# robbert-vdh/haskell-path-tracer

Measured on AMD Instinct MI355X. Metric: Msamples/sec (paths×bounces) at 1080p/64spp; achieved HBM GB/s vs peak, higher is better.
Workload: dtype f32

## Files before the change

### haskell-path-tracer_amd/_build.py

```python
import hashlib
import mmap
import os
import shutil
import subprocess
from concurrent.futures import ThreadPoolExecutor

HERE = os.path.dirname(os.path.abspath(__file__))
ROOT = os.path.dirname(HERE)
CSRC = os.path.join(HERE, "csrc")
LIB = os.path.join(HERE, "libptmi.so")
ABLATIONS_LIB = os.path.join(HERE, "libptmi_ablations.so")
OBJ_ROOT = os.path.join(ROOT, "build", "obj")
HOST_SOURCES = ["ptmi_api.cpp", "ptmi_stage.cpp", "ptmi_group.cpp", "ptmi_bvh.cpp", "ptmi_mesh.cpp"]
BUILD_ID_UNIT = "ptmi_build_id.cpp"
BUILD_ID_MARKER = b"PTMI_BUILD_ID="
SOURCE_HASH_MARKER = b"PTMI_SOURCE_HASH="
INLINE_UNIT = "ptmi_inline.hip"
KERNEL_UNITS = [INLINE_UNIT, "ptmi_streams_chain.hip", "ptmi_streams_tree.hip", "ptmi_stream_primary.hip", "ptmi_stream_pixels.hip",
                "ptmi_stream_split.hip", "ptmi_small.hip", "ptmi_mesh_refit.hip", "ptmi_mesh_build.hip", "ptmi_bvh_refit.hip", "ptmi_bvh_build.hip", "ptmi_bvh_lbvh.hip"]
ABLATION_UNITS = ["ptmi_inline_ablations.hip"]
SOURCES = HOST_SOURCES + [BUILD_ID_UNIT] + KERNEL_UNITS + ABLATION_UNITS
HEADERS = ["ptmi_core.h", "ptmi_kernels.h", "ptmi_device.h", "ptmi_bvh_device.h", "ptmi_bvh.h", "ptmi_bvh_box.h", "ptmi_bvh_spatial.h", "ptmi_mesh_device.h", "ptmi_mesh.h", "ptmi_mesh_box.h", "ptmi_mesh_morton.h", "ptmi_inline_body.inc", "ptmi_streams_chain_body.inc", "ptmi_streams_tree_body.inc", "ptmi_diag.h", "ptmi_stream_form.h", "ptmi_stage.h",
           os.path.join("..", "..", "include", "ptmi.h")]
COMPILE_FLAGS = ["--offload-arch=gfx950", "-O3", "-std=c++17", "-ffp-contract=off", "-fPIC",
                 "-fno-fast-math", "-fno-slp-vectorize", "-DPTMI_SINCOS_FUSED=1", "-Wall", "-pthread"]
LINK_FLAGS = ["--offload-arch=gfx950", "-shared", "-fPIC", "-pthread", "-ldl"]
FLAGS = COMPILE_FLAGS + ["-shared", "-ldl"]
RECIPE = "cwd=csrc,cuid=unit+flags"
JOBS = max(1, min(8, os.cpu_count() or 1))


def hipcc_path():
    for cand in (os.environ.get("HIPCC"), shutil.which("hipcc"), "/opt/rocm/bin/hipcc"):
        if cand and os.path.exists(cand):
            return cand
    raise RuntimeError("hipcc not found; libptmi.so cannot be built")


def source_hash():
    h = hashlib.sha256(" ".join(COMPILE_FLAGS + LINK_FLAGS + [RECIPE]).encode())
    for f in sorted(SOURCES + HEADERS):
        with open(os.path.join(CSRC, f), "rb") as fh:
            h.update(f.encode() + b"\0" + fh.read())
    return h.hexdigest()[:16]


def object_code_hash(obj):
    with open(obj, "rb") as fh:
        data = fh.read()
    if data[:4] != b"\x7fELF" or data[4] != 2 or data[5] != 1:
        raise RuntimeError("%s is not a little-endian ELF64 object" % obj)
    shoff = int.from_bytes(data[0x28:0x30], "little")
    shentsize, shnum, shstrndx = (int.from_bytes(data[o:o + 2], "little") for o in (0x3A, 0x3C, 0x3E))

    def header(i):
        b = data[shoff + i * shentsize: shoff + (i + 1) * shentsize]
        return (int.from_bytes(b[0:4], "little"), int.from_bytes(b[4:8], "little"), int.from_bytes(b[8:16], "little"),
                int.from_bytes(b[24:32], "little"), int.from_bytes(b[32:40], "little"))
    _, _, _, str_off, str_size = header(shstrndx)
    names = data[str_off:str_off + str_size]
    h = hashlib.sha256()
    for i in range(shnum):
        name, typ, flags, off, size = header(i)
        if not flags & 2 or typ == 8:
            continue
        h.update(names[name:names.index(b"\0", name)] + b"\0" + size.to_bytes(8, "little") + data[off:off + size])
    return h.hexdigest()


def code_id_of(objs):
    h = hashlib.sha256()
    for obj in sorted(objs, key=os.path.basename):
        h.update(os.path.basename(obj).encode() + b"\0" + object_code_hash(obj).encode() + b"\0")
    return h.hexdigest()[:16]

# ... 184 lines not shown
```

### haskell-path-tracer_amd/csrc/ptmi_core.h

```cpp
#pragma once

#include <hip/hip_runtime.h>
#include <stdint.h>

#define PTMI_HD __host__ __device__ __forceinline__

namespace ptmi {

struct V3 { float x, y, z; };
struct Quat { float w; V3 v; };
struct Sfc32 { uint32_t a, b, c, counter; };

constexpr float kPi       = 3.14159274101257324219f;
constexpr float kInfinite = 3.40282346638528859812e+38f;
constexpr float kEpsilon  = 0.002f;

PTMI_HD uint32_t f2u(float f) { return __builtin_bit_cast(uint32_t, f); }
PTMI_HD float u2f(uint32_t u) { return __builtin_bit_cast(float, u); }

PTMI_HD V3 mk(float x, float y, float z) { V3 r; r.x = x; r.y = y; r.z = z; return r; }
PTMI_HD V3 operator+(V3 a, V3 b) { return mk(a.x + b.x, a.y + b.y, a.z + b.z); }
PTMI_HD V3 operator-(V3 a, V3 b) { return mk(a.x - b.x, a.y - b.y, a.z - b.z); }
PTMI_HD V3 operator*(V3 a, V3 b) { return mk(a.x * b.x, a.y * b.y, a.z * b.z); }
PTMI_HD V3 neg(V3 a) { return mk(-a.x, -a.y, -a.z); }
PTMI_HD V3 scale_r(V3 v, float a) { return mk(v.x * a, v.y * a, v.z * a); }
PTMI_HD V3 scale_l(float a, V3 v) { return mk(a * v.x, a * v.y, a * v.z); }
PTMI_HD V3 div_r(V3 v, float a) { return mk(v.x / a, v.y / a, v.z / a); }
PTMI_HD float dot(V3 a, V3 b) { return (a.x * b.x + a.y * b.y) + a.z * b.z; }
PTMI_HD V3 cross(V3 a, V3 b)
{
    return mk(a.y * b.z - a.z * b.y, a.z * b.x - a.x * b.z, a.x * b.y - a.y * b.x);
}
PTMI_HD bool near_zero(float a) { return __builtin_fabsf(a) <= 1e-6f; }
PTMI_HD bool near_zero(V3 v) { return near_zero(dot(v, v)); }
PTMI_HD V3 normalize(V3 v)
{
    float l = dot(v, v);
    if (near_zero(l) || near_zero(1.0f - l)) return v;
    return div_r(v, __builtin_sqrtf(l));
}
PTMI_HD Quat qmul(Quat a, Quat b)
{
    Quat r;
    r.w = a.w * b.w - dot(a.v, b.v);
    r.v = (cross(a.v, b.v) + scale_l(a.w, b.v)) + scale_l(b.w, a.v);
    return r;
}
PTMI_HD V3 rotate(Quat q, V3 v)
{
    Quat qv; qv.w = 0.0f; qv.v = v;
    Quat qc; qc.w = q.w; qc.v = neg(q.v);
    return qmul(qmul(q, qv), qc).v;
}

struct Reduced { double x; int n; };
__host__ __device__ __noinline__ inline Reduced sincos_reduce_large(uint32_t xi)
{
    constexpr uint32_t inv_pio4[24] = {
        0xa2,       0xa2f9,     0xa2f983,   0xa2f9836e, 0xf9836e4e, 0x836e4e44,
        0x6e4e4415, 0x4e441529, 0x441529fc, 0x1529fc27, 0x29fc2757, 0xfc2757d1,
        0x2757d1f5, 0x57d1f534, 0xd1f534dd, 0xf534ddc0, 0x34ddc0db, 0xddc0db62,
        0xc0db6295, 0xdb629599, 0x6295993c, 0x95993c43, 0x993c4390, 0x3c439041 };
    const int base = (xi >> 26) & 15;
    const int shift = (xi >> 23) & 7;
    xi = (xi & 0xffffff) | 0x800000;
    xi <<= shift;
    uint64_t res0 = (uint32_t)(xi * inv_pio4[base]);
    uint64_t res1 = (uint64_t)xi * inv_pio4[base + 4];
    uint64_t res2 = (uint64_t)xi * inv_pio4[base + 8];
    res0 = (res2 >> 32) | (res0 << 32);
    res0 += res1;
    uint64_t n = (res0 + (1ULL << 61)) >> 62;
    res0 -= n << 62;
    Reduced r;
    r.x = (double)(int64_t)res0 * 0x1.921FB54442D18p-62;
    r.n = (int)n;
    return r;
}

PTMI_HD double local_constant(double k)
{
#if defined(__HIP_DEVICE_COMPILE__)
    uint32_t lo = (uint32_t)__builtin_bit_cast(uint64_t, k), hi = (uint32_t)(__builtin_bit_cast(uint64_t, k) >> 32);
    asm volatile("" : "+v"(lo), "+v"(hi));
    return __builtin_bit_cast(double, ((uint64_t)hi << 32) | lo);
// ... 210 lines not shown
```

### haskell-path-tracer_amd/csrc/ptmi_device.h

```cpp
#pragma once

#include "ptmi_kernels.h"
#include "ptmi_diag.h"

namespace ptmi {

namespace {

constexpr int kBlock = 256;
constexpr size_t kMaxSceneLds = 3 * 1024;
constexpr int kRenderBlock = 64;

struct HitSel { float t; int idx; bool just; };
#ifdef PTMI_NO_STAGED_WALK_OTHERS
constexpr bool kStagedWalk = false;
#else
constexpr bool kStagedWalk = true;
#endif

__device__ __forceinline__ float sqrt_rn(float x)
{
    const bool tiny = (f2u(x) - 1u) < (0x0f800000u - 1u);
    if (__builtin_expect(__any(tiny), 0)) return __builtin_sqrtf(x);
    const float s = __builtin_amdgcn_sqrtf(x);
    const float s_dn = u2f(f2u(s) - 1u), s_up = u2f(f2u(s) + 1u);
    const float e_dn = __builtin_fmaf(-s_dn, s, x);
    const float e_up = __builtin_fmaf(-s_up, s, x);
    float r = (e_dn <= 0.0f) ? s_dn : s;
    r = (e_up > 0.0f) ? s_up : r;
    return r;
}

__device__ __forceinline__ V3 div3_by_length(V3 v, float s)
{
#ifdef PTMI_PLAIN_DIVISION
    return div_r(v, s);
#else
    const float amin = __builtin_fminf(__builtin_fminf(__builtin_fabsf(v.x), __builtin_fabsf(v.y)), __builtin_fabsf(v.z));
    const bool plain = s >= 0x1p-20f && s <= 0x1p20f && amin >= 0x1p-100f;
    if (__builtin_expect(!__all(plain), 0)) return div_r(v, s);
    const float r0 = __builtin_amdgcn_rcpf(s);
    const float r = __builtin_fmaf(__builtin_fmaf(-s, r0, 1.0f), r0, r0);
    auto quotient = [&](float a) {
        float q = a * r;
        q = __builtin_fmaf(__builtin_fmaf(-s, q, a), r, q);
        return __builtin_fmaf(__builtin_fmaf(-s, q, a), r, q);
    };
    return mk(quotient(v.x), quotient(v.y), quotient(v.z));
#endif
}

template <typename ScenePtr>
__device__ __noinline__ HitSel check_hit_exact(ScenePtr S, int ns, int np, V3 o, V3 d)
{
    HitSel best; best.t = 0.0f; best.idx = 0; best.just = false;
    float best_key = 0.0f;
    for (int i = 0; i < ns + np; ++i) {
        bool just; float t;
        if (i < ns) {
            const float4 g = S[i];
            const V3 l = mk(g.x, g.y, g.z) - o;
            const float tca = dot(l, d);
            const float d2 = dot(l, l) - (tca * tca);
            const float thc = __builtin_sqrtf(g.w - d2);
            t = tca - thc;
            just = !(tca < 0.0f || d2 > g.w || t < 0.0f);
        } else {
            const float4 gp = S[ns + 2 * (i - ns)], gn = S[ns + 2 * (i - ns) + 1];
            const V3 nor = mk(gn.x, gn.y, gn.z);
            const float denom = dot(d, nor);
            t = dot(mk(gp.x, gp.y, gp.z) - o, nor) / denom;
            just = !(denom > 1e-6f || t < 0.0f);
        }
        const float key = just ? t : kInfinite;
        if (i == 0 || !(best_key <= key)) { best_key = key; best.t = t; best.idx = i; best.just = just; }
    }
    return best;
}

#define PTMI_SPHERE_TEST(g, o, d)                                                                                                   \
    const V3 l = mk(g.x, g.y, g.z) - o;                                                                                             \
    const float tca = dot(l, d);                                                                                                    \
    const float d2 = dot(l, l) - (tca * tca);                                                                                       \
    const float x = g.w - d2;                                                       \
                             \
    const bool cand = !(tca < 0.0f) && !(x < 0.0f)

template <typename At>
__device__ __forceinline__ void fold_planes(At at, int ns, int np, V3 o, V3 d, float &best_key, int &best_idx, bool &best_just,
                                            unsigned int *diag = nullptr)
{
    int stash = 0;
    float stash_denom = 1.0f;
    unsigned long long stashed = 0ull;
    auto pass = [&]() {
        diag::plane_pass(diag);
        const float4 gp = at(2 * stash), gn = at(2 * stash + 1);
        const float t = dot(mk(gp.x, gp.y, gp.z) - o, mk(gn.x, gn.y, gn.z)) / stash_denom;
        const bool just = !(stash_denom > 1e-6f) && !(t < 0.0f);
        const float key = just ? t : kInfinite;
        if (!(best_key <= key)) { best_key = key; best_idx = ns + stash; best_just = just; }
        stash_denom = 1.0f;
        stashed = 0ull;
    };
    for (int j = 0; j < np; ++j) {
        const float4 gn = at(2 * j + 1);
        const float denom = dot(d, mk(gn.x, gn.y, gn.z));
        const bool cand = !(denom > 1e-6f);
        const unsigned long long cands = __ballot(cand);
        diag::plane_test(diag);
        if (cands & stashed) pass();
        stash = cand ? j : stash;
        stash_denom = cand ? denom : stash_denom;
        stashed |= cands;
    }
    if (stashed) pass();
}

template <bool STAGED = false, typename ScenePtr>
__device__ __forceinline__ HitSel check_hit(ScenePtr S, int ns, int np, V3 o, V3 d, unsigned int *diag = nullptr)
{
    float best_key = __builtin_nanf("");
    int best_idx = 0;
    bool best_just = false;

    auto sphere = [&](const float4 g, int i) {
        PTMI_SPHERE_TEST(g, o, d);
        diag::sphere_test(diag, cand);
        if (__any(cand)) {
            const float t = tca - sqrt_rn(x);
            const bool just = cand && !(t < 0.0f);
            const float key = just ? t : kInfinite;
            if (!(best_key <= key)) { best_key = key; best_idx = i; best_just = just; }
        }
    };

    float4 ga, gb;
    int i = 0;
#if defined(__HIP_DEVICE_COMPILE__)
    typedef __attribute__((address_space(3))) const float4 *Staged;
    Staged P = nullptr;
    if constexpr (STAGED) {
        unsigned int lds_at = (unsigned int)(uintptr_t)&S[0];
        asm volatile("" : "+v"(lds_at));
        P = (Staged)(uintptr_t)lds_at;
        ga = P[0];
        for (; i + 3 < ns; i += 4) {
            gb = P[1]; sphere(ga, i);
            ga = P[2]; sphere(gb, i + 1);
            gb = P[3]; sphere(ga, i + 2);
            ga = P[4]; sphere(gb, i + 3);
            P += 4;
        }
        for (; i + 1 < ns; i += 2) {
            gb = P[1]; sphere(ga, i);
            ga = P[2]; sphere(gb, i + 1);
            P += 2;
        }
        if (i < ns) {
            sphere(ga, i);
            P += 1;
        }
    } else
#endif
    {
        ga = S[0];
        for (; i + 1 < ns; i += 2) {
            gb = S[i + 1];
            sphere(ga, i);
            ga = S[i + 2];
            sphere(gb, i + 1);
        }
        if (i < ns) sphere(ga, i);
    }
    fold_planes([&](int k) -> float4 {
#if defined(__HIP_DEVICE_COMPILE__)
        if constexpr (STAGED) return P[k]; else
#endif
        return S[ns + k];
    }, ns, np, o, d, best_key, best_idx, best_just, diag);
    if (__builtin_expect(__any(best_just && !(best_key < kInfinite)), 0))
        return check_hit_exact(S, ns, np, o, d);
    HitSel best; best.t = best_key; best.idx = best_idx; best.just = best_just;
    return best;
}

template <typename ScenePtr>
__device__ __forceinline__ void hit_record(ScenePtr S, int ns, int idx, V3 o, V3 d, float t,
                                           V3 &hit_pos, V3 &normal)
{
    hit_pos = o + scale_r(d, t);
    if (idx < ns) {
        const float4 g = S[idx];
        const V3 v = hit_pos - mk(g.x, g.y, g.z);
        const float len2 = dot(v, v);
        normal = (near_zero(len2) || near_zero(1.0f - len2)) ? v : div3_by_length(v, sqrt_rn(len2));
    } else {
        const float4 gn = S[ns + 2 * (idx - ns) + 1];
        normal = mk(gn.x, gn.y, gn.z);
    }
}

template <typename ScenePtr>
__device__ __forceinline__ V3 normal_at(ScenePtr S, int ns, int idx, V3 hit_pos)
{
    if (idx < ns) {
        const float4 g = S[idx];
        const V3 v = hit_pos - mk(g.x, g.y, g.z);
        const float len2 = dot(v, v);
        return (near_zero(len2) || near_zero(1.0f - len2)) ? v : div3_by_length(v, sqrt_rn(len2));
    }
    const float4 gn = S[ns + 2 * (idx - ns) + 1];
    return mk(gn.x, gn.y, gn.z);
}

__device__ __forceinline__ float gen_component(Sfc32 &seed)
{
    const float i = (float)(int32_t)sfc32_next(seed);
    return ((i * 4.656612873077392578125e-10f + 1.0f) + 2.3283064365386962890625e-10f) - 1.0f;
}

__device__ __forceinline__ void bounce_axis(float4 mb, V3 normal, V3 d, V3 &axis, float &hk)
{
    const bool matte = f2u(mb.x) == 0u;
    const float ia = dot(d, normal);
    const V3 reflection = d - scale_l(2.0f * ia, normal);
    axis = matte ? normal : reflection;
    hk = matte ? 0.5f * kPi : mb.w;
}

__device__ __forceinline__ void next_about_axis(float4 mb, V3 axis, float hk, Sfc32 &seed, V3 &next, float &brdf)
{
    const bool matte = f2u(mb.x) == 0u;
    V3 rv;
    rv.x = gen_component(seed); rv.y = gen_component(seed); rv.z = gen_component(seed);
    next = rotate(quaternion_from_half_angles(hk * rv.x, hk * rv.y, hk * rv.z), axis);
    const float nd = dot(next, axis);
    brdf = matte ? mb.z * nd : __builtin_fmaxf(0.0f, nd);
}

// ... 276 lines not shown
```

### haskell-path-tracer_amd/csrc/ptmi_inline.hip

```cpp
#include "ptmi_mesh_device.h"

namespace ptmi {

namespace {

#ifndef PTMI_INLINE_WAVES
#define PTMI_INLINE_WAVES 7
#endif
template <bool LDS_SCENE, int TILE_W = 0>
__global__ void __launch_bounds__(kRenderBlock, PTMI_INLINE_WAVES) render_inline_kernel(const RenderArgs a)
{
#define PTMI_HIT(STAGED, ...) check_hit<STAGED>(__VA_ARGS__)
#define PTMI_HIT_RECORD hit_record
#define PTMI_NORMAL_AT normal_at
#include "ptmi_inline_body.inc"
#undef PTMI_HIT_RECORD
#undef PTMI_NORMAL_AT
#undef PTMI_HIT
}

#ifndef PTMI_CONTRACTED_BUILD
template <int TILE_W>
__global__ void __launch_bounds__(kRenderBlock, PTMI_BVH_WAVES) render_inline_bvh_kernel(const RenderArgs a, const BvhView bvh)
{
    constexpr bool LDS_SCENE = false;
#define PTMI_HIT(STAGED, S, ns, np, o, d, ...) check_hit_bvh(bvh, S, ns, np, o, d)
#define PTMI_HIT_RECORD hit_record
#define PTMI_NORMAL_AT normal_at
#include "ptmi_inline_body.inc"
#undef PTMI_HIT_RECORD
#undef PTMI_NORMAL_AT
#undef PTMI_HIT
}

template <int TILE_W>
__global__ void __launch_bounds__(kRenderBlock, PTMI_BVH_WAVES) render_inline_mesh_kernel(const RenderArgs a, const MeshView mesh)
{
    constexpr bool LDS_SCENE = false;
#define PTMI_HIT(STAGED, S, ns, np, o, d, ...) check_hit_mesh(mesh, S, ns, np, o, d)
#define PTMI_HIT_RECORD(S, ns, idx, o, d, t, p, n) mesh_hit_record(mesh, S, ns, np, idx, o, d, t, p, n)
#define PTMI_NORMAL_AT(S, ns, idx, p) mesh_normal_at(mesh, S, ns, np, idx, p)
#include "ptmi_inline_body.inc"
#undef PTMI_HIT_RECORD
#undef PTMI_NORMAL_AT
#undef PTMI_HIT
}
#endif

hipError_t launch_linear(const RenderArgs &a, Mapping mapping, bool lds_scene, hipStream_t stream)
{
    if (lds_scene) return launch_per_pixel(a, mapping, render_inline_kernel<true, 8>, render_inline_kernel<true>, true, PTMI_INLINE_WAVES, 16, stream);
    return launch_per_pixel(a, mapping, render_inline_kernel<false, 8>, render_inline_kernel<false>, false, PTMI_INLINE_WAVES, 16, stream);
}

}

hipError_t launch_render_inline(const RenderArgs &a, const BvhView *bvh, int variant, hipStream_t stream)
{
    if (renders_nothing(a)) return hipSuccess;
#ifndef PTMI_CONTRACTED_BUILD
    if (bvh) return launch_per_pixel(a, Mapping::kAuto, render_inline_bvh_kernel<8>, render_inline_bvh_kernel<0>, false, PTMI_BVH_WAVES, 16, stream, *bvh);
#endif
    const bool lds_scene = scene_fits_lds(a);
    if (variant == kVariantAuto || a.bounce_limit <= 0 || a.n_spp <= 0) return launch_linear(a, Mapping::kAuto, lds_scene, stream);
    if (!lds_scene) {
        if (variant == kVariantPersistent) variant = kVariantPersistentScalar;
        else if (variant == kVariantRows || variant == kVariantCapped4 || variant == kVariantCapped3) variant = kVariantRowsScalar;
        else if (variant >= kVariantTiles && variant <= kVariantTiles32x2) variant = kVariantTilesScalar;
// ... 55 lines not shown
```

### haskell-path-tracer_amd/csrc/ptmi_inline_body.inc

```
    __shared__ float pixel_const[10][kRenderBlock];
    extern __shared__ float4 lds_scene[];
    const int ns = a.scene.n_spheres, np = a.scene.n_planes;
    if (LDS_SCENE) {
        const int total = a.scene.total_f4();
        for (int i = threadIdx.x; i < total; i += kRenderBlock) lds_scene[i] = a.scene.packed[i];
        __syncthreads();
    }
    const float4 *S = LDS_SCENE ? lds_scene : a.scene.packed;
    const float4 *M = S + a.scene.geom_f4();

    unsigned int wg; int chunk, n_spp_chunk;
    enter_sample_chunk<TILE_W>(a, wg, chunk, n_spp_chunk);
    long long pixel;
    unsigned int quad, trips = 0;
    const bool valid = lane_pixel<TILE_W>(a, pixel, quad, wg);
    unsigned int live = 0;
    if (valid) {
        const int local_row = (int)(pixel / a.width);
        const int col = (int)(pixel - (long long)local_row * a.width);
        int64_t px = col, py = global_row(local_row, a.stripe_rows, a.n_parts, a.part);
        if (a.screen_x) { px = a.screen_x[pixel]; py = a.screen_y[pixel]; }

        const V3 origin = a.cam.pos;
        const V3 primary = primary_direction(a.cam, px, py);

        V3 acc = mk(a.planes.r[pixel], a.planes.g[pixel], a.planes.b[pixel]);
        Sfc32 seed;
        seed.a = a.planes.sa[pixel]; seed.b = a.planes.sb[pixel];
        seed.c = a.planes.sc[pixel]; seed.counter = a.planes.sctr[pixel];

        const int limit = a.bounce_limit, n_spp = n_spp_chunk;

        if (limit <= 0) {
            if (n_spp > 0) acc = mk(0.0f, 0.0f, 0.0f) + acc;
        } else {
            const HitSel h0 = PTMI_HIT(LDS_SCENE, S, ns, np, origin, primary);
            if (!h0.just) {
                if (n_spp > 0) acc = mk(0.0f, 0.0f, 0.0f) + acc;
            } else {
                float *mine = &pixel_const[0][threadIdx.x];
                auto put = [&](int k, float v) { mine[k * kRenderBlock] = v; };
                auto get = [&](int k) { return mine[k * kRenderBlock]; };
                V3 pos, normal;
                PTMI_HIT_RECORD(S, ns, h0.idx, origin, primary, h0.t, pos, normal);
                const int idx0 = h0.idx;
                {
                    const float4 mb0 = M[2 * idx0 + 1];
                    V3 axis0; float hk0;
                    bounce_axis(mb0, normal, primary, axis0, hk0);
                    put(0, pos.x); put(1, pos.y); put(2, pos.z);
                    put(3, axis0.x); put(4, axis0.y); put(5, axis0.z); put(6, hk0);
                    put(7, acc.x); put(8, acc.y); put(9, acc.z);
                }
                int s = -1, it = 0, idx = idx0;
                V3 d = primary;
                V3 throughput = mk(1.0f, 1.0f, 1.0f), result = mk(0.0f, 0.0f, 0.0f);
                bool pending = false, has_ray = false, over = n_spp > 0;
                diag::PhaseProbe phase;
                while (pending || over) {
                    ++trips;
                    phase.trip(); phase.round_a(pending || over);
                    float4 mb = M[2 * idx + 1];
                    V3 axis = mk(0.0f, 0.0f, 0.0f); float hk = 0.0f;
                    phase.check(pending);
                    if (pending) {
                        bounce_axis(mb, normal, d, axis, hk);
                        const float4 ma = M[2 * idx];
                        if (it + 1 >= limit || surely_frozen_after(ma, mb, axis, throughput)) {
                            finish_frozen(ma, throughput, result, seed);
                            ++live;
                            phase.frozen();
                            pending = false; over = true;
                        }
                    }
                    phase.restart(over);
                    if (over) {
                        if (s >= 0) { put(7, result.x + get(7)); put(8, result.y + get(8)); put(9, result.z + get(9)); }
                        ++s; it = 0;
                        throughput = mk(1.0f, 1.0f, 1.0f); result = mk(0.0f, 0.0f, 0.0f);
                        pos = mk(get(0), get(1), get(2)); idx = idx0;
                        mb = M[2 * idx0 + 1];
                        axis = mk(get(3), get(4), get(5)); hk = get(6);
                        over = false; pending = s < n_spp;
                    }
                    phase.shade(pending);
                    if (pending) {
                        V3 next; float brdf;
                        sincos3_probe(a.work_counter, hk, seed);
                        next_about_axis(mb, axis, hk, seed, next, brdf);
                        apply_bounce(M, idx, pos, next, brdf, pos, d, throughput, result);
                        ++it; ++live;
                        pending = false;
                        if (it >= limit || near_zero(throughput)) over = true;
                        else has_ray = true;
                    }
                    phase.end_a(); phase.round_c(has_ray);
                    if (has_ray) {
                        const HitSel h = PTMI_HIT(LDS_SCENE, S, ns, np, pos, d, diag::sphere_counters(a.work_counter));
                        has_ray = false;
                        if (h.just) {
                            PTMI_HIT_RECORD(S, ns, h.idx, pos, d, h.t, pos, normal);
                            idx = h.idx;
                            pending = true;
                        } else {
                            over = true;
                        }
                    }
                    phase.end_c();
                }
                acc = mk(get(7), get(8), get(9));
                phase.flush(a.work_counter);
            }
        }

        a.planes.r[pixel] = acc.x; a.planes.g[pixel] = acc.y; a.planes.b[pixel] = acc.z;
        a.planes.sa[pixel] = seed.a; a.planes.sb[pixel] = seed.b;
        a.planes.sc[pixel] = seed.c; a.planes.sctr[pixel] = seed.counter;
    }
    leave_sample_chunk<TILE_W>(a, wg, chunk);

    if (TILE_W > 0) record_cost(a, quad, trips);
    if (a.live_counter) {
        const unsigned long long total = wave_sum(live);
        if ((threadIdx.x & 63) == 0 && total) atomicAdd(a.live_counter + (size_t)(blockIdx.x & (kStatShards - 1)) * kStatStride, total);
    }
```

### haskell-path-tracer_amd/csrc/ptmi_small.hip

```cpp
#include "ptmi_mesh_device.h"

namespace ptmi {

namespace {

__global__ void __launch_bounds__(kBlock) seed_kernel(Planes p, int width, int rows_local, int stripe_rows,
                                                      int n_parts, int part, uint64_t seed0, int clear_color)
{
    const long long n_local = (long long)rows_local * width;
    const long long pixel = (long long)blockIdx.x * kBlock + threadIdx.x;
    if (pixel >= n_local) return;
    const int local_row = (int)(pixel / width);
    const int col = (int)(pixel - (long long)local_row * width);
    const uint64_t index = (uint64_t)global_row(local_row, stripe_rows, n_parts, part) * (uint64_t)width + (uint64_t)col;
    const Sfc32 s = sfc32_seed3(seed_word(seed0, index, 0), seed_word(seed0, index, 1), seed_word(seed0, index, 2));
    p.sa[pixel] = s.a; p.sb[pixel] = s.b; p.sc[pixel] = s.c; p.sctr[pixel] = s.counter;
    if (clear_color) { p.r[pixel] = 0.0f; p.g[pixel] = 0.0f; p.b[pixel] = 0.0f; }
}

__global__ void __launch_bounds__(kBlock) create_with_kernel(Planes p, const uint32_t *w0, const uint32_t *w1,
                                                             const uint32_t *w2, long long n)
{
    const long long i = (long long)blockIdx.x * kBlock + threadIdx.x;
    if (i >= n) return;
// ... 32 lines not shown
            o[2] = float4{b[2], r[3], g[3], b[3]};
        }
        if (rgba) {
            uint4 v;
            v.x = unorm8(r[0]) | unorm8(g[0]) << 8 | unorm8(b[0]) << 16 | 0xff000000u;
            v.y = unorm8(r[1]) | unorm8(g[1]) << 8 | unorm8(b[1]) << 16 | 0xff000000u;
            v.z = unorm8(r[2]) | unorm8(g[2]) << 8 | unorm8(b[2]) << 16 | 0xff000000u;
            v.w = unorm8(r[3]) | unorm8(g[3]) << 8 | unorm8(b[3]) << 16 | 0xff000000u;
            *reinterpret_cast<uint4 *>(rgba + q) = v;
        }
    } else {
        for (int k = 0; k < 4 && q + k < n; ++k) {
            if (rgb) { rgb[3 * (q + k)] = r[k]; rgb[3 * (q + k) + 1] = g[k]; rgb[3 * (q + k) + 2] = b[k]; }
            if (rgba) rgba[q + k] = unorm8(r[k]) | unorm8(g[k]) << 8 | unorm8(b[k]) << 16 | 0xff000000u;
        }
    }
}

__global__ void __launch_bounds__(kBlock) stitch_kernel(const float *src, int rows, int width, int stripe_rows, int n_parts, int part,
                                                        float *r, float *g, float *b)
{
    const long long n = (long long)rows * width;
    const long long i = (long long)blockIdx.x * kBlock + threadIdx.x;
    if (i >= n) return;
    const int local_row = (int)(i / width);
    const int col = (int)(i - (long long)local_row * width);
    const long long o = (long long)global_row(local_row, stripe_rows, n_parts, part) * width + col;
    r[o] = src[i]; g[o] = src[n + i]; b[o] = src[2 * n + i];
}

__global__ void __launch_bounds__(kBlock) eval_sphere_kernel(const float *sph, const float *rays, int n,
                                                             int32_t *is_just, float *t_out, float *normalp)
{
    const int i = blockIdx.x * kBlock + threadIdx.x;
    if (i >= n) return;
    const float *s = sph + 10 * (size_t)i;
    float4 g[2]; g[0].x = s[0]; g[0].y = s[1]; g[0].z = s[2]; g[0].w = s[3] * s[3];
    g[1] = g[0];
    const V3 o = mk(rays[6 * i], rays[6 * i + 1], rays[6 * i + 2]);
    const V3 d = mk(rays[6 * i + 3], rays[6 * i + 4], rays[6 * i + 5]);
    const HitSel h = check_hit(g, 1, 0, o, d);
    is_just[i] = h.just ? 1 : 0;
    t_out[i] = h.just ? h.t : 0.0f;
    if (normalp) {
        V3 hp = mk(0, 0, 0), nr = mk(0, 0, 0);
        if (h.just) hit_record(g, 1, 0, o, d, h.t, hp, nr);
        float *q = normalp + 6 * (size_t)i;
        q[0] = hp.x; q[1] = hp.y; q[2] = hp.z; q[3] = nr.x; q[4] = nr.y; q[5] = nr.z;
    }
}

template <bool BVH>
__global__ void __launch_bounds__(kRenderBlock) eval_check_hit_kernel(const SceneView scene, const BvhView bvh, const float *rays, int n,
                                                                      float *t_out, int32_t *idx_out, int32_t *just_out)
{
    const int i = blockIdx.x * kRenderBlock + threadIdx.x;
    if (i >= n) return;
    const V3 o = mk(rays[6 * (size_t)i], rays[6 * (size_t)i + 1], rays[6 * (size_t)i + 2]);
    const V3 d = mk(rays[6 * (size_t)i + 3], rays[6 * (size_t)i + 4], rays[6 * (size_t)i + 5]);
    const HitSel h = BVH ? check_hit_bvh(bvh, scene.packed, scene.n_spheres, scene.n_planes, o, d)
                         : check_hit(scene.packed, scene.n_spheres, scene.n_planes, o, d);
    just_out[i] = h.just ? 1 : 0;
    t_out[i] = h.just ? h.t : 0.0f;
    idx_out[i] = h.just ? h.idx : -1;
}

__global__ void __launch_bounds__(kRenderBlock) eval_check_hit_mesh_kernel(const SceneView scene, const MeshView mesh, const float *rays, int n,
                                                                           float *t_out, int32_t *idx_out, int32_t *just_out)
{
    const int i = blockIdx.x * kRenderBlock + threadIdx.x;
    if (i >= n) return;
    const V3 o = mk(rays[6 * (size_t)i], rays[6 * (size_t)i + 1], rays[6 * (size_t)i + 2]);
    const V3 d = mk(rays[6 * (size_t)i + 3], rays[6 * (size_t)i + 4], rays[6 * (size_t)i + 5]);
    const HitSel h = check_hit_mesh(mesh, scene.packed, scene.n_spheres, scene.n_planes, o, d);
    just_out[i] = h.just ? 1 : 0;
    t_out[i] = h.just ? h.t : 0.0f;
    idx_out[i] = h.just ? h.idx : -1;
}

__global__ void __launch_bounds__(kBlock) eval_plane_kernel(const float *pl, const float *rays, int n,
                                                            int32_t *is_just, float *t_out, float *normalp)
{
    const int i = blockIdx.x * kBlock + threadIdx.x;
    if (i >= n) return;
    const float *s = pl + 12 * (size_t)i;
    float4 g[3];
    g[0].x = s[0]; g[0].y = s[1]; g[0].z = s[2]; g[0].w = 0.0f;
    g[1].x = s[3]; g[1].y = s[4]; g[1].z = s[5]; g[1].w = 0.0f;
    g[2] = g[0];
    const V3 o = mk(rays[6 * i], rays[6 * i + 1], rays[6 * i + 2]);
    const V3 d = mk(rays[6 * i + 3], rays[6 * i + 4], rays[6 * i + 5]);
    const HitSel h = check_hit(g, 0, 1, o, d);
    is_just[i] = h.just ? 1 : 0;
    t_out[i] = h.just ? h.t : 0.0f;
    if (normalp) {
        V3 hp = mk(0, 0, 0), nr = mk(0, 0, 0);
        if (h.just) hit_record(g, 0, 0, o, d, h.t, hp, nr);
        float *q = normalp + 6 * (size_t)i;
        q[0] = hp.x; q[1] = hp.y; q[2] = hp.z; q[3] = nr.x; q[4] = nr.y; q[5] = nr.z;
    }
}

__global__ void __launch_bounds__(kBlock) eval_sincos_kernel(const float *x, int n, float *s, float *c)
{
    const int i = blockIdx.x * kBlock + threadIdx.x;
    if (i >= n) return;
    float sn, cs;
    sincos(x[i], sn, cs);
    s[i] = sn; c[i] = cs;
// ... 40 lines not shown
            unsigned int t = (cut < 256 && total) ? start[cut] : n;
            t = (t + 7u) & ~7u;
            *tail_start = t < n ? t : n;
        }
    }
    __syncthreads();
    for (unsigned int i = threadIdx.x; i < n; i += 1024) order[atomicAdd(&start[cls[i]], 1u)] = i;
}

}

bool uses_quad_order(const RenderArgs &a, int algorithm_inline, int variant)
{
    if (variant != kVariantAuto || !tiles_pay(a) || a.screen_x) return false;
    return algorithm_inline ? (a.bounce_limit > 0 && a.n_spp > 0) : true;
}


hipError_t launch_quad_order(const unsigned int *cost, unsigned int *order, unsigned int *cls, unsigned int n, unsigned int *tail_start,
                             unsigned int tail_permille, hipStream_t stream)
{
    if (n == 0) return hipSuccess;
    return launch(quad_order_kernel, dim3(1), dim3(1024), 0, stream, cost, order, cls, n, tail_start, tail_permille);
}


hipError_t launch_seed(Planes p, int width, int rows_local, int stripe_rows, int n_parts, int part,
                       uint64_t seed0, bool clear_color, hipStream_t stream)
{
    const long long n = (long long)rows_local * width;
    if (n <= 0) return hipSuccess;
    return launch(seed_kernel, dim3(blocks_for(n)), dim3(kBlock), 0, stream, p, width, rows_local,
                  stripe_rows, n_parts, part, seed0, clear_color ? 1 : 0);
}

hipError_t launch_create_with(Planes p, const uint32_t *w0, const uint32_t *w1, const uint32_t *w2,
                              int64_t n, hipStream_t stream)
{
    if (n <= 0) return hipSuccess;
    return launch(create_with_kernel, dim3(blocks_for(n)), dim3(kBlock), 0, stream, p, w0, w1, w2, (long long)n);
}

hipError_t launch_eval_sphere(const float *spheres10, const float *rays, int n,
                              int32_t *is_just, float *t, float *normalp, hipStream_t stream)
{
    if (n <= 0) return hipSuccess;
    return launch(eval_sphere_kernel, dim3(blocks_for(n)), dim3(kBlock), 0, stream, spheres10, rays, n, is_just, t, normalp);
}

hipError_t launch_eval_check_hit(SceneView scene, const BvhView *bvh, const float *rays, int n, float *t, int32_t *idx, int32_t *just, hipStream_t stream)
{
    if (n <= 0) return hipSuccess;
    const dim3 grid(blocks_for(n, kRenderBlock)), block(kRenderBlock);
    if (bvh) return launch(eval_check_hit_kernel<true>, grid, block, 0, stream, scene, *bvh, rays, n, t, idx, just);
    return launch(eval_check_hit_kernel<false>, grid, block, 0, stream, scene, BvhView{}, rays, n, t, idx, just);
}

hipError_t launch_eval_check_hit_mesh(SceneView scene, const MeshView &mesh, const float *rays, int n, float *t, int32_t *idx, int32_t *just, hipStream_t stream)
{
    if (n <= 0) return hipSuccess;
    return launch(eval_check_hit_mesh_kernel, dim3(blocks_for(n, kRenderBlock)), dim3(kRenderBlock), 0, stream, scene, mesh, rays, n, t, idx, just);
}

hipError_t launch_eval_plane(const float *planes12, const float *rays, int n,
                             int32_t *is_just, float *t, float *normalp, hipStream_t stream)
{
    if (n <= 0) return hipSuccess;
    return launch(eval_plane_kernel, dim3(blocks_for(n)), dim3(kBlock), 0, stream, planes12, rays, n, is_just, t, normalp);
}

hipError_t launch_present(Planes p, long long n, int iterations, float *rgb, uint32_t *rgba, hipStream_t stream)
{
    if (n <= 0) return hipSuccess;
    const uintptr_t bits = (uintptr_t)p.r | (uintptr_t)p.g | (uintptr_t)p.b | (uintptr_t)rgb | (uintptr_t)rgba;
    return launch(present_kernel, dim3(blocks_for((n + 3) / 4)), dim3(kBlock), 0, stream, p, n, (float)iterations, rgb, rgba,
                  (bits & 15u) == 0 ? 1 : 0);
}

hipError_t launch_stitch(const float *src, int rows, int width, int stripe_rows, int n_parts, int part,
                         float *r, float *g, float *b, hipStream_t stream)
{
    const long long n = (long long)rows * width;
    if (n <= 0) return hipSuccess;
    return launch(stitch_kernel, dim3(blocks_for(n)), dim3(kBlock), 0, stream, src, rows, width, stripe_rows, n_parts, part, r, g, b);
}

hipError_t launch_eval_sincos(const float *x, int n, float *s, float *c, hipStream_t stream)
{
    if (n <= 0) return hipSuccess;
    return launch(eval_sincos_kernel, dim3(blocks_for(n)), dim3(kBlock), 0, stream, x, n, s, c);
}

hipError_t launch_eval_quaternion(const float *half_angles, int n, float *q_out, hipStream_t stream)
{
    if (n <= 0) return hipSuccess;
    return launch(eval_quaternion_kernel, dim3(blocks_for(n)), dim3(kBlock), 0, stream, half_angles, n, q_out);
}


}
```

Measured before the change: 392,100.

## Add wave-wide MFMA sphere culling vote before per-ray sphere tests

Adds a conservative sphere culling pass that uses MFMA 16x16x4 f32 matrix ops to evaluate, for each sphere (up to 16), whether any ray in the wave could hit it. Only spheres the wave votes for are then tested per ray, with a fallback to the exact path when precision bounds are not met. The inline kernel's bounce loop is restructured into a wave-uniform loop so the wave-level vote can run each trip. The aim is to cut per-ray sphere intersection ALU work, at the cost of extra MFMA, permlane and ballot work every trip and possibly more divergence handling.

```diff
diff --git a/haskell-path-tracer_amd/_build.py b/haskell-path-tracer_amd/_build.py
--- a/haskell-path-tracer_amd/_build.py
+++ b/haskell-path-tracer_amd/_build.py
@@ -20,7 +20,7 @@
                 "ptmi_stream_split.hip", "ptmi_small.hip", "ptmi_mesh_refit.hip", "ptmi_mesh_build.hip", "ptmi_bvh_refit.hip", "ptmi_bvh_build.hip", "ptmi_bvh_lbvh.hip"]
 ABLATION_UNITS = ["ptmi_inline_ablations.hip"]
 SOURCES = HOST_SOURCES + [BUILD_ID_UNIT] + KERNEL_UNITS + ABLATION_UNITS
-HEADERS = ["ptmi_core.h", "ptmi_kernels.h", "ptmi_device.h", "ptmi_bvh_device.h", "ptmi_bvh.h", "ptmi_bvh_box.h", "ptmi_bvh_spatial.h", "ptmi_mesh_device.h", "ptmi_mesh.h", "ptmi_mesh_box.h", "ptmi_mesh_morton.h", "ptmi_inline_body.inc", "ptmi_streams_chain_body.inc", "ptmi_streams_tree_body.inc", "ptmi_diag.h", "ptmi_stream_form.h", "ptmi_stage.h",
+HEADERS = ["ptmi_core.h", "ptmi_kernels.h", "ptmi_device.h", "ptmi_bvh_device.h", "ptmi_bvh.h", "ptmi_bvh_box.h", "ptmi_bvh_spatial.h", "ptmi_mesh_device.h", "ptmi_mesh.h", "ptmi_mesh_box.h", "ptmi_mesh_morton.h", "ptmi_inline_body.inc", "ptmi_inline_trip.inc", "ptmi_sphere_cull.h", "ptmi_streams_chain_body.inc", "ptmi_streams_tree_body.inc", "ptmi_diag.h", "ptmi_stream_form.h", "ptmi_stage.h",
            os.path.join("..", "..", "include", "ptmi.h")]
 COMPILE_FLAGS = ["--offload-arch=gfx950", "-O3", "-std=c++17", "-ffp-contract=off", "-fPIC",
                  "-fno-fast-math", "-fno-slp-vectorize", "-DPTMI_SINCOS_FUSED=1", "-Wall", "-pthread"]
diff --git a/haskell-path-tracer_amd/csrc/ptmi_core.h b/haskell-path-tracer_amd/csrc/ptmi_core.h
--- a/haskell-path-tracer_amd/csrc/ptmi_core.h
+++ b/haskell-path-tracer_amd/csrc/ptmi_core.h
@@ -31,6 +31,14 @@
 {
     return mk(a.y * b.z - a.z * b.y, a.z * b.x - a.x * b.z, a.x * b.y - a.y * b.x);
 }
+#define PTMI_SPHERE_TEST(g, o, d)                                                                                                   \
+    const V3 l = mk(g.x, g.y, g.z) - o;                                                                                             \
+    const float tca = dot(l, d);                                                                                                    \
+    const float d2 = dot(l, l) - (tca * tca);                                                                                       \
+    const float x = g.w - d2;                                                       \
+                             \
+    const bool cand = !(tca < 0.0f) && !(x < 0.0f)
+
 PTMI_HD bool near_zero(float a) { return __builtin_fabsf(a) <= 1e-6f; }
 PTMI_HD bool near_zero(V3 v) { return near_zero(dot(v, v)); }
 PTMI_HD V3 normalize(V3 v)
diff --git a/haskell-path-tracer_amd/csrc/ptmi_device.h b/haskell-path-tracer_amd/csrc/ptmi_device.h
--- a/haskell-path-tracer_amd/csrc/ptmi_device.h
+++ b/haskell-path-tracer_amd/csrc/ptmi_device.h
@@ -2,6 +2,7 @@
 
 #include "ptmi_kernels.h"
 #include "ptmi_diag.h"
+#include "ptmi_sphere_cull.h"
 
 namespace ptmi {
 
@@ -78,13 +79,6 @@
     return best;
 }
 
-#define PTMI_SPHERE_TEST(g, o, d)                                                                                                   \
-    const V3 l = mk(g.x, g.y, g.z) - o;                                                                                             \
-    const float tca = dot(l, d);                                                                                                    \
-    const float d2 = dot(l, l) - (tca * tca);                                                                                       \
-    const float x = g.w - d2;                                                       \
-                             \
-    const bool cand = !(tca < 0.0f) && !(x < 0.0f)
 
 template <typename At>
 __device__ __forceinline__ void fold_planes(At at, int ns, int np, V3 o, V3 d, float &best_key, int &best_idx, bool &best_just,
@@ -186,6 +180,33 @@
 }
 
 template <typename ScenePtr>
+__device__ __forceinline__ HitSel check_hit_survivors(ScenePtr S, int ns, int np, V3 o, V3 d, unsigned int survivors, unsigned int *diag = nullptr)
+{
+    float best_key = __builtin_nanf("");
+    int best_idx = 0;
+    bool best_just = false;
+    unsigned int left = __builtin_amdgcn_readfirstlane(survivors);
+    while (left) {
+        const int i = __builtin_ctz(left);
+        left &= left - 1u;
+        const float4 g = S[i];
+        PTMI_SPHERE_TEST(g, o, d);
+        diag::sphere_test(diag, cand);
+        if (__any(cand)) {
+            const float t = tca - sqrt_rn(x);
+            const bool just = cand && !(t < 0.0f);
+            const float key = just ? t : kInfinite;
+            if (!(best_key <= key)) { best_key = key; best_idx = i; best_just = just; }
+        }
+    }
+    fold_planes([&](int k) -> float4 { return S[ns + k]; }, ns, np, o, d, best_key, best_idx, best_just, diag);
+    if (__builtin_expect(__any(best_just && !(best_key < kInfinite)), 0))
+        return check_hit_exact(S, ns, np, o, d);
+    HitSel best; best.t = best_key; best.idx = best_idx; best.just = best_just;
+    return best;
+}
+
+template <typename ScenePtr>
 __device__ __forceinline__ void hit_record(ScenePtr S, int ns, int idx, V3 o, V3 d, float t,
                                            V3 &hit_pos, V3 &normal)
 {
diff --git a/haskell-path-tracer_amd/csrc/ptmi_inline.hip b/haskell-path-tracer_amd/csrc/ptmi_inline.hip
--- a/haskell-path-tracer_amd/csrc/ptmi_inline.hip
+++ b/haskell-path-tracer_amd/csrc/ptmi_inline.hip
@@ -13,7 +13,20 @@
 #define PTMI_HIT(STAGED, ...) check_hit<STAGED>(__VA_ARGS__)
 #define PTMI_HIT_RECORD hit_record
 #define PTMI_NORMAL_AT normal_at
+#ifndef PTMI_NESTED_LOOP
+#define PTMI_UNIFORM_LOOP
+#if !defined(PTMI_CONTRACTED_BUILD) && !defined(PTMI_NO_SPHERE_CULL)
+#define PTMI_SPHERE_CULL
+#define PTMI_TRACE_VOTE(o, d, has_ray) const unsigned int cull_vote = sphere_cull_vote(S, ns, cull_scene, o, d, has_ray)
+#define PTMI_HIT_BOUNCE(STAGED, S, ns, np, o, d, dg) \
+    ((cull_vote & kCullRefused) ? check_hit<STAGED>(S, ns, np, o, d, dg) : check_hit_survivors(S, ns, np, o, d, cull_vote, dg))
+#endif
+#endif
 #include "ptmi_inline_body.inc"
+#undef PTMI_TRACE_VOTE
+#undef PTMI_HIT_BOUNCE
+#undef PTMI_SPHERE_CULL
+#undef PTMI_UNIFORM_LOOP
 #undef PTMI_HIT_RECORD
 #undef PTMI_NORMAL_AT
 #undef PTMI_HIT
diff --git a/haskell-path-tracer_amd/csrc/ptmi_inline_body.inc b/haskell-path-tracer_amd/csrc/ptmi_inline_body.inc
--- a/haskell-path-tracer_amd/csrc/ptmi_inline_body.inc
+++ b/haskell-path-tracer_amd/csrc/ptmi_inline_body.inc
@@ -1,3 +1,11 @@
+#ifndef PTMI_TRACE_VOTE
+#define PTMI_TRACE_VOTE(o, d, has_ray)
+#define PTMI_TRACE_VOTE_DEFAULTED
+#endif
+#ifndef PTMI_HIT_BOUNCE
+#define PTMI_HIT_BOUNCE PTMI_HIT
+#define PTMI_HIT_BOUNCE_DEFAULTED
+#endif
     __shared__ float pixel_const[10][kRenderBlock];
     extern __shared__ float4 lds_scene[];
     const int ns = a.scene.n_spheres, np = a.scene.n_planes;
@@ -8,12 +16,81 @@
     }
     const float4 *S = LDS_SCENE ? lds_scene : a.scene.packed;
     const float4 *M = S + a.scene.geom_f4();
+#ifdef PTMI_SPHERE_CULL
+    CullScene cull_scene = cull_scene_none();
+    if (LDS_SCENE && ns >= 1 && ns <= kCullSpheres) cull_scene = cull_stage(S, ns);
+#endif
 
     unsigned int wg; int chunk, n_spp_chunk;
     enter_sample_chunk<TILE_W>(a, wg, chunk, n_spp_chunk);
     long long pixel;
     unsigned int quad, trips = 0;
     const bool valid = lane_pixel<TILE_W>(a, pixel, quad, wg);
+#ifdef PTMI_UNIFORM_LOOP
+    unsigned int live = 0;
+    const int limit = a.bounce_limit, n_spp = n_spp_chunk;
+    V3 acc = mk(0.0f, 0.0f, 0.0f);
+    Sfc32 seed; seed.a = seed.b = seed.c = seed.counter = 0u;
+    float *mine = &pixel_const[0][threadIdx.x];
+    auto put = [&](int k, float v) { mine[k * kRenderBlock] = v; };
+    auto get = [&](int k) { return mine[k * kRenderBlock]; };
+    V3 pos = mk(0.0f, 0.0f, 0.0f), normal = mk(0.0f, 0.0f, 0.0f), d = mk(0.0f, 0.0f, 1.0f);
+    int idx0 = 0;
+    bool run = false;
+    if (valid) {
+        const int local_row = (int)(pixel / a.width);
+        const int col = (int)(pixel - (long long)local_row * a.width);
+        int64_t px = col, py = global_row(local_row, a.stripe_rows, a.n_parts, a.part);
+        if (a.screen_x) { px = a.screen_x[pixel]; py = a.screen_y[pixel]; }
+
+        const V3 origin = a.cam.pos;
+        const V3 primary = primary_direction(a.cam, px, py);
+
+        acc = mk(a.planes.r[pixel], a.planes.g[pixel], a.planes.b[pixel]);
+        seed.a = a.planes.sa[pixel]; seed.b = a.planes.sb[pixel];
+        seed.c = a.planes.sc[pixel]; seed.counter = a.planes.sctr[pixel];
+
+        if (limit <= 0) {
+            if (n_spp > 0) acc = mk(0.0f, 0.0f, 0.0f) + acc;
+        } else {
+            const HitSel h0 = PTMI_HIT(LDS_SCENE, S, ns, np, origin, primary);
+            if (!h0.just) {
+                if (n_spp > 0) acc = mk(0.0f, 0.0f, 0.0f) + acc;
+            } else {
+                PTMI_HIT_RECORD(S, ns, h0.idx, origin, primary, h0.t, pos, normal);
+                idx0 = h0.idx;
+                const float4 mb0 = M[2 * idx0 + 1];
+                V3 axis0; float hk0;
+                bounce_axis(mb0, normal, primary, axis0, hk0);
+                put(0, pos.x); put(1, pos.y); put(2, pos.z);
+                put(3, axis0.x); put(4, axis0.y); put(5, axis0.z); put(6, hk0);
+                put(7, acc.x); put(8, acc.y); put(9, acc.z);
+                d = primary;
+                run = true;
+            }
+        }
+    }
+    {
+        int s = -1, it = 0, idx = idx0;
+        V3 throughput = mk(1.0f, 1.0f, 1.0f), result = mk(0.0f, 0.0f, 0.0f);
+        bool pending = false, has_ray = false, over = run && n_spp > 0;
+        diag::PhaseProbe phase;
+        while (__any(pending || over)) {
+            if (pending || over) { ++trips; phase.trip(); }
+            phase.round_a(pending || over);
+#include "ptmi_inline_trip.inc"
+        }
+        if (run) {
+            acc = mk(get(7), get(8), get(9));
+            phase.flush(a.work_counter);
+        }
+    }
+    if (valid) {
+        a.planes.r[pixel] = acc.x; a.planes.g[pixel] = acc.y; a.planes.b[pixel] = acc.z;
+        a.planes.sa[pixel] = seed.a; a.planes.sb[pixel] = seed.b;
+        a.planes.sc[pixel] = seed.c; a.planes.sctr[pixel] = seed.counter;
+    }
+#else
     unsigned int live = 0;
     if (valid) {
         const int local_row = (int)(pixel / a.width);
@@ -60,53 +137,7 @@
                 while (pending || over) {
                     ++trips;
                     phase.trip(); phase.round_a(pending || over);
-                    float4 mb = M[2 * idx + 1];
-                    V3 axis = mk(0.0f, 0.0f, 0.0f); float hk = 0.0f;
-                    phase.check(pending);
-                    if (pending) {
-                        bounce_axis(mb, normal, d, axis, hk);
-                        const float4 ma = M[2 * idx];
-                        if (it + 1 >= limit || surely_frozen_after(ma, mb, axis, throughput)) {
-                            finish_frozen(ma, throughput, result, seed);
-                            ++live;
-                            phase.frozen();
-                            pending = false; over = true;
-                        }
-                    }
-                    phase.restart(over);
-                    if (over) {
-                        if (s >= 0) { put(7, result.x + get(7)); put(8, result.y + get(8)); put(9, result.z + get(9)); }
-                        ++s; it = 0;
-                        throughput = mk(1.0f, 1.0f, 1.0f); result = mk(0.0f, 0.0f, 0.0f);
-                        pos = mk(get(0), get(1), get(2)); idx = idx0;
-                        mb = M[2 * idx0 + 1];
-                        axis = mk(get(3), get(4), get(5)); hk = get(6);
-                        over = false; pending = s < n_spp;
-                    }
-                    phase.shade(pending);
-                    if (pending) {
-                        V3 next; float brdf;
-                        sincos3_probe(a.work_counter, hk, seed);
-                        next_about_axis(mb, axis, hk, seed, next, brdf);
-                        apply_bounce(M, idx, pos, next, brdf, pos, d, throughput, result);
-                        ++it; ++live;
-                        pending = false;
-                        if (it >= limit || near_zero(throughput)) over = true;
-                        else has_ray = true;
-                    }
-                    phase.end_a(); phase.round_c(has_ray);
-                    if (has_ray) {
-                        const HitSel h = PTMI_HIT(LDS_SCENE, S, ns, np, pos, d, diag::sphere_counters(a.work_counter));
-                        has_ray = false;
-                        if (h.just) {
-                            PTMI_HIT_RECORD(S, ns, h.idx, pos, d, h.t, pos, normal);
-                            idx = h.idx;
-                            pending = true;
-                        } else {
-                            over = true;
-                        }
-                    }
-                    phase.end_c();
+#include "ptmi_inline_trip.inc"
                 }
                 acc = mk(get(7), get(8), get(9));
                 phase.flush(a.work_counter);
@@ -117,6 +148,7 @@
         a.planes.sa[pixel] = seed.a; a.planes.sb[pixel] = seed.b;
         a.planes.sc[pixel] = seed.c; a.planes.sctr[pixel] = seed.counter;
     }
+#endif
     leave_sample_chunk<TILE_W>(a, wg, chunk);
 
     if (TILE_W > 0) record_cost(a, quad, trips);
@@ -124,3 +156,11 @@
         const unsigned long long total = wave_sum(live);
         if ((threadIdx.x & 63) == 0 && total) atomicAdd(a.live_counter + (size_t)(blockIdx.x & (kStatShards - 1)) * kStatStride, total);
     }
+#ifdef PTMI_TRACE_VOTE_DEFAULTED
+#undef PTMI_TRACE_VOTE
+#undef PTMI_TRACE_VOTE_DEFAULTED
+#endif
+#ifdef PTMI_HIT_BOUNCE_DEFAULTED
+#undef PTMI_HIT_BOUNCE
+#undef PTMI_HIT_BOUNCE_DEFAULTED
+#endif
diff --git a/haskell-path-tracer_amd/csrc/ptmi_inline_trip.inc b/haskell-path-tracer_amd/csrc/ptmi_inline_trip.inc
--- /dev/null
+++ b/haskell-path-tracer_amd/csrc/ptmi_inline_trip.inc
@@ -0,0 +1,48 @@
+                    float4 mb = M[2 * idx + 1];
+                    V3 axis = mk(0.0f, 0.0f, 0.0f); float hk = 0.0f;
+                    phase.check(pending);
+                    if (pending) {
+                        bounce_axis(mb, normal, d, axis, hk);
+                        const float4 ma = M[2 * idx];
+                        if (it + 1 >= limit || surely_frozen_after(ma, mb, axis, throughput)) {
+                            finish_frozen(ma, throughput, result, seed);
+                            ++live;
+                            phase.frozen();
+                            pending = false; over = true;
+                        }
+                    }
+                    phase.restart(over);
+                    if (over) {
+                        if (s >= 0) { put(7, result.x + get(7)); put(8, result.y + get(8)); put(9, result.z + get(9)); }
+                        ++s; it = 0;
+                        throughput = mk(1.0f, 1.0f, 1.0f); result = mk(0.0f, 0.0f, 0.0f);
+                        pos = mk(get(0), get(1), get(2)); idx = idx0;
+                        mb = M[2 * idx0 + 1];
+                        axis = mk(get(3), get(4), get(5)); hk = get(6);
+                        over = false; pending = s < n_spp;
+                    }
+                    phase.shade(pending);
+                    if (pending) {
+                        V3 next; float brdf;
+                        sincos3_probe(a.work_counter, hk, seed);
+                        next_about_axis(mb, axis, hk, seed, next, brdf);
+                        apply_bounce(M, idx, pos, next, brdf, pos, d, throughput, result);
+                        ++it; ++live;
+                        pending = false;
+                        if (it >= limit || near_zero(throughput)) over = true;
+                        else has_ray = true;
+                    }
+                    phase.end_a(); phase.round_c(has_ray);
+                    PTMI_TRACE_VOTE(pos, d, has_ray);
+                    if (has_ray) {
+                        const HitSel h = PTMI_HIT_BOUNCE(LDS_SCENE, S, ns, np, pos, d, diag::sphere_counters(a.work_counter));
+                        has_ray = false;
+                        if (h.just) {
+                            PTMI_HIT_RECORD(S, ns, h.idx, pos, d, h.t, pos, normal);
+                            idx = h.idx;
+                            pending = true;
+                        } else {
+                            over = true;
+                        }
+                    }
+                    phase.end_c();
diff --git a/haskell-path-tracer_amd/csrc/ptmi_small.hip b/haskell-path-tracer_amd/csrc/ptmi_small.hip
--- a/haskell-path-tracer_amd/csrc/ptmi_small.hip
+++ b/haskell-path-tracer_amd/csrc/ptmi_small.hip
@@ -108,9 +108,33 @@
 
 template <bool BVH>
 __global__ void __launch_bounds__(kRenderBlock) eval_check_hit_kernel(const SceneView scene, const BvhView bvh, const float *rays, int n,
-                                                                      float *t_out, int32_t *idx_out, int32_t *just_out)
+                                                                      float *t_out, int32_t *idx_out, int32_t *just_out, int culled)
 {
     const int i = blockIdx.x * kRenderBlock + threadIdx.x;
+    if constexpr (!BVH) {
+        if (culled) {
+            extern __shared__ float4 lds_scene[];
+            const int ns = scene.n_spheres, np = scene.n_planes, geom = scene.geom_f4();
+            for (int k = threadIdx.x; k < geom; k += kRenderBlock) lds_scene[k] = scene.packed[k];
+            __syncthreads();
+            const CullScene cull_scene = cull_stage(lds_scene, ns);
+            const bool active = i < n;
+            V3 o = mk(0.0f, 0.0f, 0.0f), d = mk(0.0f, 0.0f, 1.0f);
+            if (active) {
+                o = mk(rays[6 * (size_t)i], rays[6 * (size_t)i + 1], rays[6 * (size_t)i + 2]);
+                d = mk(rays[6 * (size_t)i + 3], rays[6 * (size_t)i + 4], rays[6 * (size_t)i + 5]);
+            }
+            const unsigned int vote = sphere_cull_vote(lds_scene, ns, cull_scene, o, d, active);
+            if (active) {
+                const HitSel h = (vote & kCullRefused) ? check_hit(scene.packed, ns, np, o, d)
+                                                       : check_hit_survivors((const float4 *)lds_scene, ns, np, o, d, vote);
+                just_out[i] = h.just ? 1 : 0;
+                t_out[i] = h.just ? h.t : 0.0f;
+                idx_out[i] = h.just ? h.idx : -1;
+            }
+            return;
+        }
+    }
     if (i >= n) return;
     const V3 o = mk(rays[6 * (size_t)i], rays[6 * (size_t)i + 1], rays[6 * (size_t)i + 2]);
     const V3 d = mk(rays[6 * (size_t)i + 3], rays[6 * (size_t)i + 4], rays[6 * (size_t)i + 5]);
@@ -257,8 +281,10 @@
 {
     if (n <= 0) return hipSuccess;
     const dim3 grid(blocks_for(n, kRenderBlock)), block(kRenderBlock);
-    if (bvh) return launch(eval_check_hit_kernel<true>, grid, block, 0, stream, scene, *bvh, rays, n, t, idx, just);
-    return launch(eval_check_hit_kernel<false>, grid, block, 0, stream, scene, BvhView{}, rays, n, t, idx, just);
+    if (bvh) return launch(eval_check_hit_kernel<true>, grid, block, 0, stream, scene, *bvh, rays, n, t, idx, just, 0);
+    const size_t geom = (size_t)scene.geom_f4() * sizeof(float4);
+    const bool culled = scene.n_spheres >= 1 && scene.n_spheres <= kCullSpheres && geom <= kMaxSceneLds;
+    return launch(eval_check_hit_kernel<false>, grid, block, culled ? geom : 0, stream, scene, BvhView{}, rays, n, t, idx, just, culled ? 1 : 0);
 }
 
 hipError_t launch_eval_check_hit_mesh(SceneView scene, const MeshView &mesh, const float *rays, int n, float *t, int32_t *idx, int32_t *just, hipStream_t stream)
diff --git a/haskell-path-tracer_amd/csrc/ptmi_sphere_cull.h b/haskell-path-tracer_amd/csrc/ptmi_sphere_cull.h
--- /dev/null
+++ b/haskell-path-tracer_amd/csrc/ptmi_sphere_cull.h
@@ -0,0 +1,134 @@
+#pragma once
+
+#include "ptmi_core.h"
+
+namespace ptmi {
+
+constexpr int kCullSpheres = 16;
+constexpr float kCullCoordBound = 0x1p40f;
+constexpr float kCullR2Bound = 0x1p80f;
+constexpr float kCullD1Min = 0.5f, kCullD1Max = 2.5f;
+constexpr float kCullMarginT = 0x1p-19f, kCullMarginX = 0x1p-18f, kCullFloor = 0x1p-100f;
+constexpr float kCullReject = 0x1p100f;
+constexpr unsigned int kCullRefused = 0x80000000u;
+
+struct CullScene { float cmax, gmax; bool ok; };
+
+PTMI_HD CullScene cull_scene_none() { CullScene s; s.cmax = 0.0f; s.gmax = 0.0f; s.ok = false; return s; }
+
+PTMI_HD void cull_scene_add(CullScene &s, float4 g)
+{
+    const float c = __builtin_fmaxf(__builtin_fmaxf(__builtin_fabsf(g.x), __builtin_fabsf(g.y)), __builtin_fabsf(g.z));
+    const bool fine = __builtin_fabsf(g.x) <= kCullCoordBound && __builtin_fabsf(g.y) <= kCullCoordBound && __builtin_fabsf(g.z) <= kCullCoordBound &&
+                      __builtin_fabsf(g.w) <= kCullR2Bound;
+    s.ok = s.ok && fine;
+    s.cmax = __builtin_fmaxf(s.cmax, c);
+    s.gmax = __builtin_fmaxf(s.gmax, __builtin_fabsf(g.w));
+}
+
+PTMI_HD float cull_a1(float4 g, int k) { return k == 0 ? -g.x : k == 1 ? -g.y : k == 2 ? -g.z : 1.0f; }
+PTMI_HD float cull_a2(float4 g, int k) { return k == 0 ? -2.0f * g.x : k == 1 ? -2.0f * g.y : k == 2 ? -2.0f * g.z : -1.0f; }
+PTMI_HD float cull_c(float4 g) { return dot(mk(g.x, g.y, g.z), mk(g.x, g.y, g.z)) - g.w; }
+
+struct CullRay { float q, p; bool ok; };
+
+PTMI_HD CullRay cull_ray_terms(V3 o, V3 d, float cmax, float gmax)
+{
+    const float o1 = (__builtin_fabsf(o.x) + __builtin_fabsf(o.y)) + __builtin_fabsf(o.z);
+    const float d1 = (__builtin_fabsf(d.x) + __builtin_fabsf(d.y)) + __builtin_fabsf(d.z);
+    const float r = cmax + o1, w = r * d1;
+    const float m_t = __builtin_fmaf(kCullMarginT, w, kCullFloor);
+    const float big = __builtin_fmaf(w, w, __builtin_fmaf(3.0f, r * r, gmax));
+    const float m_x = __builtin_fmaf(kCullMarginX, big, kCullFloor);
+    const float od = __builtin_fmaf(o.x, d.x, __builtin_fmaf(o.y, d.y, o.z * d.z));
+    const float oo = __builtin_fmaf(o.x, o.x, __builtin_fmaf(o.y, o.y, o.z * o.z));
+    CullRay t;
+    t.q = od - m_t;
+    t.p = m_x - oo;
+    t.ok = o1 < kCullCoordBound && d1 > kCullD1Min && d1 < kCullD1Max;
+    return t;
+}
+
+PTMI_HD bool cull_pair_passes(float4 g, V3 o, V3 d, CullRay t)
+{
+    const float b1[4] = {d.x, d.y, d.z, t.q}, b2[4] = {o.x, o.y, o.z, t.p};
+    float s = 0.0f, n = cull_c(g);
+    for (int k = 0; k < 4; ++k) {
+        s = __builtin_fmaf(cull_a1(g, k), b1[k], s);
+        n = __builtin_fmaf(cull_a2(g, k), b2[k], n);
+    }
+    const float xn = __builtin_fmaf(-s, s, n);
+    return ((f2u(s) & f2u(xn)) >> 31) != 0u;
+}
+
+#if defined(__HIPCC__)
+namespace {
+
+typedef float CullAcc __attribute__((ext_vector_type(4)));
+
+template <typename ScenePtr>
+__device__ __forceinline__ CullScene cull_stage(ScenePtr S, int ns)
+{
+    CullScene s; s.cmax = 0.0f; s.gmax = 0.0f; s.ok = true;
+    for (int j = 0; j < ns; ++j) cull_scene_add(s, S[j]);
+    s.cmax = u2f(__builtin_amdgcn_readfirstlane(f2u(s.cmax)));
+    s.gmax = u2f(__builtin_amdgcn_readfirstlane(f2u(s.gmax)));
+    s.ok = __builtin_amdgcn_readfirstlane(s.ok ? 1 : 0) != 0;
+    return s;
+}
+
+__device__ __forceinline__ void cull_transpose(float (&v)[4])
+{
+    auto swap16 = [](float &x, float &y) {
+        const auto r = __builtin_amdgcn_permlane16_swap(f2u(x), f2u(y), false, false);
+        x = u2f(r[0]); y = u2f(r[1]);
+    };
+    auto swap32 = [](float &x, float &y) {
+        const auto r = __builtin_amdgcn_permlane32_swap(f2u(x), f2u(y), false, false);
+        x = u2f(r[0]); y = u2f(r[1]);
+    };
+    swap16(v[0], v[1]); swap16(v[2], v[3]);
+    swap32(v[0], v[2]); swap32(v[1], v[3]);
+}
+
+__device__ __forceinline__ unsigned int sphere_cull_vote(const float4 *S, int ns, CullScene scene, V3 o, V3 d, bool active)
+{
+    if (!scene.ok) return kCullRefused;
+    const CullRay t = cull_ray_terms(o, d, scene.cmax, scene.gmax);
+    if (__builtin_expect(!__all(t.ok || !active), 0)) return kCullRefused;
+    float b1[4] = {d.x, d.y, d.z, active ? t.q : kCullReject};
+    float b2[4] = {o.x, o.y, o.z, t.p};
+    cull_transpose(b1);
+    cull_transpose(b2);
+    const int lane = threadIdx.x & 63, k = lane >> 4, last = ns - 1;
+    const float v = reinterpret_cast<const float *>(S)[4 * min(lane & 15, last) + k];
+    const float a1 = k == 3 ? 1.0f : -v, a2 = k == 3 ? -1.0f : -2.0f * v;
+    const float c_mine = cull_c(S[min(4 * k + (lane & 3), last)]);
+    CullAcc c;
+    c[0] = u2f(__builtin_amdgcn_update_dpp(0u, f2u(c_mine), 0x150, 0xf, 0xf, false));
+    c[1] = u2f(__builtin_amdgcn_update_dpp(0u, f2u(c_mine), 0x151, 0xf, 0xf, false));
+    c[2] = u2f(__builtin_amdgcn_update_dpp(0u, f2u(c_mine), 0x152, 0xf, 0xf, false));
+    c[3] = u2f(__builtin_amdgcn_update_dpp(0u, f2u(c_mine), 0x153, 0xf, 0xf, false));
+    const CullAcc zero = {0.0f, 0.0f, 0.0f, 0.0f};
+    unsigned int both[4] = {0u, 0u, 0u, 0u};
+#pragma unroll
+    for (int g = 0; g < 4; ++g) {
+        const CullAcc s = __builtin_amdgcn_mfma_f32_16x16x4f32(a1, b1[g], zero, 0, 0, 0);
+        const CullAcc n = __builtin_amdgcn_mfma_f32_16x16x4f32(a2, b2[g], c, 0, 0, 0);
+#pragma unroll
+        for (int r = 0; r < 4; ++r) both[r] |= f2u(s[r]) & f2u(__builtin_fmaf(-s[r], s[r], n[r]));
+    }
+    unsigned int mask = 0u;
+#pragma unroll
+    for (int r = 0; r < 4; ++r) {
+        const unsigned long long m = __ballot((int)both[r] < 0);
+#pragma unroll
+        for (int q = 0; q < 4; ++q) mask |= ((m >> (16 * q)) & 0xffffull) ? 1u << (4 * q + r) : 0u;
+    }
+    return mask & ((1u << ns) - 1u);
+}
+
+}
+#endif
+
+}
```

After: 337,600. -13.9%, worse.
